# chen-bowen/instacart_next_order_recommendation

Measured on NVIDIA B200. Metric: top-k queries/sec (IR-eval batch: 10,000 queries x 49,688x384 fp32 catalog, top-100), higher is better.
Workload: dtype f32

## Files before the change

### instacart_next_order_recommendation_b200/csrc/gemm_topk.cu

```cuda
#include "select_args.cuh"
#include "select_lean.cuh"
#include "select_finish.cuh"
#include "tc.cuh"

namespace icr {

constexpr int kRingBytes = 192 * 1024;
constexpr int kSegCapMax = 512;
#ifndef ICR_EPI_WARPS_F32
#define ICR_EPI_WARPS_F32 4
#endif
#ifndef ICR_EPI_WARPS_BF16
#define ICR_EPI_WARPS_BF16 8
#endif
__host__ __device__ constexpr int epi_warps(int terms) { return terms == 3 ? ICR_EPI_WARPS_F32 : ICR_EPI_WARPS_BF16; }
constexpr int kEpiWarps = 8;
constexpr int kEpiCols = BN;
constexpr int kGemmThreads = 128 + kEpiWarps * 32;
constexpr int kTmemCols = 512;
constexpr int kMaxStages = 6;
constexpr int kAStatMaxKB = 6;

struct GemmArgs {
  int Q, N;
  int k;
  int kb_per_term;
  int plane_stride;
  int tile_begin, tile_end;
  int chunks;
  int qblocks;
  float acc_scale;
  const float* tau;
  const float* qinv;
// ... 91 lines not shown

template <bool BF16>
__device__ __forceinline__ void filter32(const uint32_t (&r)[32], SegState& s, const float* cinv32, float cmax, float cmin, int rbase,
                                         bool fast, int N, const uint8_t* mask) {
  const float tau_f = unorder_bits(s.tau_ob);
  if (fast) {
    float m[16];
#pragma unroll
    for (int j = 0; j < 16; ++j) m[j] = fmaxf(__uint_as_float(r[2 * j]), __uint_as_float(r[2 * j + 1]));
#pragma unroll
    for (int w = 8; w > 0; w >>= 1)
#pragma unroll
      for (int j = 0; j < w; ++j) m[j] = fmaxf(m[j], m[j + w]);
    const float bound = BF16 ? fmaxf(m[0] * cmax, m[0] * cmin) : m[0];
    if (__any_sync(kFull, bound > tau_f)) {
      float sc[32];
      if (BF16) {
#pragma unroll
        for (int j = 0; j < 32; j += 4) {
          const float4 ci = *reinterpret_cast<const float4*>(cinv32 + j);
          sc[j] = __uint_as_float(r[j]) * ci.x;
          sc[j + 1] = __uint_as_float(r[j + 1]) * ci.y;
          sc[j + 2] = __uint_as_float(r[j + 2]) * ci.z;
          sc[j + 3] = __uint_as_float(r[j + 3]) * ci.w;
        }
      } else {
#pragma unroll
        for (int j = 0; j < 32; ++j) sc[j] = __uint_as_float(r[j]);
      }
      int off[33];
      off[0] = s.cnt;
#pragma unroll
      for (int g = 0; g < 4; ++g) {
        int inc[8];
#pragma unroll
        for (int j = 0; j < 8; ++j) inc[j] = (sc[g * 8 + j] > tau_f) ? 1 : 0;
        const int s01 = inc[0] + inc[1], s23 = inc[2] + inc[3], s45 = inc[4] + inc[5], s67 = inc[6] + inc[7];
        const int b = off[g * 8];
        off[g * 8 + 1] = b + inc[0];
        off[g * 8 + 2] = b + s01;
        off[g * 8 + 3] = b + s01 + inc[2];
        const int b4 = b + s01 + s23;
        off[g * 8 + 4] = b4;
        off[g * 8 + 5] = b4 + inc[4];
        off[g * 8 + 6] = b4 + s45;
        off[g * 8 + 7] = b4 + s45 + inc[6];
        off[g * 8 + 8] = b4 + s45 + s67;
      }
      const uint32_t nrow0 = ~static_cast<uint32_t>(rbase);
#pragma unroll
      for (int j = 0; j < 32; ++j) {
        asm volatile(
            "{\n"
            ".reg .pred p;\n"
            "setp.gt.f32 p, %1, %2;\n"
            "@p st.global.v2.u32 [%0], {%3, %4};\n"
            "}\n" ::"l"(s.seg + off[j]),
            "f"(sc[j]), "f"(tau_f), "r"(nrow0 - j), "r"(__float_as_uint(sc[j]))
            : "memory");
      }
      s.cnt = off[32];
    }
  } else {
#pragma unroll
    for (int j = 0; j < 32; ++j) {
      const int row = rbase + j;
      if (row < N && !(mask && mask[row])) {
        const float sc = BF16 ? __uint_as_float(r[j]) * cinv32[j] : __uint_as_float(r[j]);
        append_if(s, sc, tau_f, ~static_cast<uint32_t>(row));
      }
    }
  }
}

template <bool BF16>
__device__ __forceinline__ void dense_store32(const uint32_t (&r)[32], float* out_row, float qscale, const float* cinv32, int ncols,
// ... 21 lines not shown
    unsigned long long t0, t1;
    asm volatile("mov.u64 %0, %%globaltimer;" : "=l"(t0));
    for (;;) {
      unsigned int v;
      asm volatile("ld.acquire.gpu.global.u32 %0, [%1];" : "=r"(v) : "l"(counter) : "memory");
      if (v >= ctas) break;
      __nanosleep(100);
      asm volatile("mov.u64 %0, %%globaltimer;" : "=l"(t1));
      if (t1 - t0 > 2000000000ull) __trap();
    }
    __threadfence();
  }
  asm volatile("bar.sync 2, %0;" ::"r"(ewarps * 32) : "memory");
}

template <int MODE, bool ASTAT, bool DENSE>
__global__ void __cluster_dims__(2, 1, 1) __launch_bounds__(kGemmThreads, 1)
gemm_topk_kernel(const __grid_constant__ CUtensorMap tma_a, const __grid_constant__ CUtensorMap tma_b, const GemmArgs g) {
  constexpr int TERMS = (MODE == 3) ? 3 : 1;
  static_assert(!ASTAT || TERMS == 1, "A-stationary is a one-term variant");
  constexpr bool BF16 = (MODE == 1);
  constexpr int EW = epi_warps(TERMS), EH = EW / 4, ECOLS = BN / EH;
  constexpr int kStageTiles = ASTAT ? 1 : ((TERMS == 3) ? 4 : 2);
  constexpr int kStageBytes = kStageTiles * kTileBytes;
  constexpr int kAResidentBytes = ASTAT ? kAStatMaxKB * kTileBytes : 0;
  constexpr int kStages = (kRingBytes - kAResidentBytes) / kStageBytes;
  static_assert(kStages <= kMaxStages, "barrier array too small");

  extern __shared__ __align__(1024) unsigned char smem_raw[];
  unsigned char* smem = smem_raw + ((1024u - (smem_u32(smem_raw) & 1023u)) & 1023u);
  unsigned char* a_resident = smem;
  unsigned char* stage_base = smem + kAResidentBytes;
  float* cinv_all = reinterpret_cast<float*>(smem + kRingBytes);
  uint64_t* bars = reinterpret_cast<uint64_t*>(cinv_all + EW * ECOLS);
  uint64_t* full_bar = bars;
  uint64_t* empty_bar = bars + kMaxStages;
  uint64_t* tfull_bar = bars + 2 * kMaxStages;
  uint64_t* tempty_bar = bars + 2 * kMaxStages + 2;
  uint64_t* afull_bar = bars + 2 * kMaxStages + 4;
  uint64_t* aempty_bar = bars + 2 * kMaxStages + 5;
  uint32_t* tmem_ptr = reinterpret_cast<uint32_t*>(bars + 2 * kMaxStages + 6);
  uint32_t* boot_s = reinterpret_cast<uint32_t*>(bars + 2 * kMaxStages + 7);

  const int warp = threadIdx.x >> 5, lane = threadIdx.x & 31;
  const uint32_t rank = cluster_ctarank();
  const int pair = blockIdx.x >> 1, npairs = gridDim.x >> 1;
  const int KB = g.kb_per_term;
  const int items = g.qblocks * g.chunks;

  if (threadIdx.x == 0) {
    for (int s = 0; s < kStages; ++s) {
      mbar_init(smem_u32(&full_bar[s]), 1);
      mbar_init(smem_u32(&empty_bar[s]), 1);
    }
    for (int a = 0; a < 2; ++a) {
      mbar_init(smem_u32(&tfull_bar[a]), 1);
      mbar_init(smem_u32(&tempty_bar[a]), 2 * EW);
    }
    mbar_init(smem_u32(afull_bar), 1);
    mbar_init(smem_u32(aempty_bar), 1);
    asm volatile("fence.mbarrier_init.release.cluster;" ::: "memory");
    asm volatile("prefetch.tensormap [%0];" ::"l"(&tma_a) : "memory");
    asm volatile("prefetch.tensormap [%0];" ::"l"(&tma_b) : "memory");
  }
  if (warp == 2) tmem_alloc_pair(smem_u32(tmem_ptr), kTmemCols);
  tc_fence_before();
  __syncthreads();
  cluster_sync_all();
  tc_fence_after();
  const uint32_t tmem_base = *tmem_ptr;

  if (warp == 0 && lane == 0) {
    int stage = 0;
    uint32_t phase = 0, a_phase = 0;
    for (int pass = g.boot > 0 ? 0 : 1; pass < 2; ++pass)
    for (int w = pair; w < items; w += npairs) {
      const int chunk = w / g.qblocks, qb = w - chunk * g.qblocks;
      const int t0 = chunk_first_tile(g, chunk), t1 = pass == 0 ? t0 + g.boot : chunk_first_tile(g, chunk + 1);
      const int qrow = qb * (2 * BM) + static_cast<int>(rank) * BM;
      if (ASTAT) {
        mbar_wait(smem_u32(aempty_bar), a_phase ^ 1);
        const uint32_t ab = smem_u32(afull_bar);
        if (rank == 0) mbar_expect_tx(ab, 2 * KB * kTileBytes);
        for (int kb = 0; kb < KB; ++kb) tma_load_2d_pair(smem_u32(a_resident + kb * kTileBytes), &tma_a, kb * BK, qrow, ab);
        a_phase ^= 1;
      }
      for (int tile = t0; tile < t1; ++tile) {
        const int crow = tile * BN + static_cast<int>(rank) * BNH;
        for (int kb = 0; kb < KB; ++kb) {
          mbar_wait(smem_u32(&empty_bar[stage]), phase ^ 1);
          const uint32_t fb = smem_u32(&full_bar[stage]);
          if (rank == 0) mbar_expect_tx(fb, 2 * kStageBytes);
          const uint32_t sa = smem_u32(stage_base + stage * kStageBytes);
          if (ASTAT) {
            tma_load_2d_pair(sa, &tma_b, kb * BK, crow, fb);
          } else if (TERMS == 3) {
            tma_load_2d_pair(sa, &tma_a, kb * BK, qrow, fb);
            tma_load_2d_pair(sa + kTileBytes, &tma_a, g.plane_stride + kb * BK, qrow, fb);
            tma_load_2d_pair(sa + 2 * kTileBytes, &tma_b, kb * BK, crow, fb);
            tma_load_2d_pair(sa + 3 * kTileBytes, &tma_b, g.plane_stride + kb * BK, crow, fb);
          } else {
            tma_load_2d_pair(sa, &tma_a, kb * BK, qrow, fb);
            tma_load_2d_pair(sa + kTileBytes, &tma_b, kb * BK, crow, fb);
          }
          if (++stage == kStages) {
            stage = 0;
            phase ^= 1;
          }
        }
      }
    }
  } else if (warp == 1 && rank == 0) {
    const uint32_t fmt = BF16 ? 1u : 0u;
    const uint32_t idesc = (1u << 4) | (fmt << 7) | (fmt << 10) | (static_cast<uint32_t>(BN >> 3) << 17) | (static_cast<uint32_t>((2 * BM) >> 4) << 24);
    const uint64_t a_res0 = smem_desc_sw128(smem_u32(a_resident));
    const uint64_t st0 = smem_desc_sw128(smem_u32(stage_base));
    constexpr uint64_t kTileUnits = kTileBytes >> 4, kStageUnits = kStageBytes >> 4;
    int stage = 0;
    uint32_t phase = 0;
    int acc = 0;
    uint32_t acc_phase = 0, a_phase = 0;
    for (int pass = g.boot > 0 ? 0 : 1; pass < 2; ++pass)
    for (int w = pair; w < items; w += npairs) {
      const int chunk = w / g.qblocks;
      const int t0 = chunk_first_tile(g, chunk), t1 = pass == 0 ? t0 + g.boot : chunk_first_tile(g, chunk + 1);
      if (ASTAT) {
        mbar_wait(smem_u32(afull_bar), a_phase);
        tc_fence_after();
        a_phase ^= 1;
      }
      for (int tile = t0; tile < t1; ++tile) {
        mbar_wait(smem_u32(&tempty_bar[acc]), acc_phase ^ 1);
        tc_fence_after();
        const uint32_t d_tmem = tmem_base + static_cast<uint32_t>(acc * BN);
        for (int kb = 0; kb < KB; ++kb) {
          mbar_wait(smem_u32(&full_bar[stage]), phase);
          tc_fence_after();
          const uint64_t sd = st0 + static_cast<uint64_t>(stage) * kStageUnits;
          if (elect_one()) {
            if (ASTAT) {
              const uint64_t adesc = a_res0 + static_cast<uint64_t>(kb) * kTileUnits, bdesc = sd;
#pragma unroll
              for (int k4 = 0; k4 < BK / 16; ++k4) {
                const uint64_t o = static_cast<uint64_t>(k4 * 2);
                umma_f16_pair(d_tmem, adesc + o, bdesc + o, idesc, (kb | k4) != 0 ? 1u : 0u);
              }
            } else if (TERMS == 3) {
              const uint64_t a_hi = sd, a_lo = sd + kTileUnits, b_hi = sd + 2 * kTileUnits, b_lo = sd + 3 * kTileUnits;
#pragma unroll
              for (int k4 = 0; k4 < BK / 16; ++k4) {
                const uint64_t o = static_cast<uint64_t>(k4 * 2);
                umma_f16_pair(d_tmem, a_hi + o, b_hi + o, idesc, (kb | k4) != 0 ? 1u : 0u);
                umma_f16_pair(d_tmem, a_hi + o, b_lo + o, idesc, 1u);
                umma_f16_pair(d_tmem, a_lo + o, b_hi + o, idesc, 1u);
              }
            } else {
              const uint64_t adesc = sd, bdesc = sd + kTileUnits;
#pragma unroll
              for (int k4 = 0; k4 < BK / 16; ++k4) {
                const uint64_t o = static_cast<uint64_t>(k4 * 2);
                umma_f16_pair(d_tmem, adesc + o, bdesc + o, idesc, (kb | k4) != 0 ? 1u : 0u);
              }
            }
            umma_commit_pair(smem_u32(&empty_bar[stage]));
            if (kb == KB - 1) umma_commit_pair(smem_u32(&tfull_bar[acc]));
          }
          __syncwarp();
          if (++stage == kStages) {
            stage = 0;
            phase ^= 1;
          }
        }
        if (++acc == 2) {
          acc = 0;
          acc_phase ^= 1;
        }
      }
      if (ASTAT) {
        if (elect_one()) umma_commit_pair(smem_u32(aempty_bar));
        __syncwarp();
      }
    }
  } else if (warp >= 4 && warp < 4 + EW) {
    const int ew = (warp - 4) & 3;
    const int half = (warp - 4) >> 2;
    uint64_t* scratch = g.compact_scratch + (static_cast<int64_t>(blockIdx.x) * EW + (warp - 4)) * kSegCapMax;
    float* cinv_s = cinv_all + (warp - 4) * ECOLS;
    const int cap = g.seg_cap;
    int acc = 0;
    uint32_t acc_phase = 0;
    if (!DENSE && g.boot > 0) {
      const int per_tile = g.boot_coarse ? 1 : (ECOLS / 32);
      const int gstride = g.chunks * g.boot * EH * per_tile;
      for (int w = pair; w < items; w += npairs) {
        const int chunk = w / g.qblocks, qb = w - chunk * g.qblocks;
        const int t0 = chunk_first_tile(g, chunk);
        const int q = qb * (2 * BM) + static_cast<int>(rank) * BM + ew * 32 + lane;
        const bool live = q < g.Q;
        float* gq = g.gmax + static_cast<int64_t>(live ? q : 0) * gstride + (chunk * g.boot * EH + half) * per_tile;
        for (int bt = 0; bt < g.boot; ++bt) {
          float m_tile = -INFINITY;
          const int row0 = (t0 + bt) * BN + half * ECOLS;
// ... 28 lines not shown
              }
            }
            m_tile = fmaxf(m_tile, m);
            if (live && !g.boot_coarse) gq[bt * (EH * (ECOLS / 32)) + cb] = m;
          }
          if (live && g.boot_coarse) gq[bt * EH] = m_tile;
          tc_fence_before();
          __syncwarp();
          if (lane == 0) mbar_arrive_cluster(smem_u32(&tempty_bar[acc]), 0);
          if (++acc == 2) {
            acc = 0;
            acc_phase ^= 1;
          }
        }
      }
      k2_grid_barrier(g.gsync, gridDim.x, warp - 4, EW);
      uint32_t* bsc = boot_s + (warp - 4) * (kK2BootCap + kHsBins);
      uint32_t* bhist = bsc + kK2BootCap;
      const int nwarps = static_cast<int>(gridDim.x) * EW;
      for (int j = blockIdx.x * EW + (warp - 4); j < g.Q; j += nwarps) {
        for (int i = lane; i < gstride; i += 32) bsc[i] = order_bits(__ldcg(g.gmax + static_cast<int64_t>(j) * gstride + i));
        __syncwarp();
        uint32_t ks, kr;
        ls_kth(bsc, bsc, gstride, g.k, bhist, lane, ks, kr);
        if (lane == 0) const_cast<float*>(g.tau)[j] = unorder_bits(ks > 1u ? ks - 1u : ks) - g.band;
        __syncwarp();
      }
      k2_grid_barrier(g.gsync + 1, gridDim.x, warp - 4, EW);
    }
    for (int w = pair; w < items; w += npairs) {
      const int chunk = w / g.qblocks, qb = w - chunk * g.qblocks;
      const int t0 = chunk_first_tile(g, chunk), t1 = chunk_first_tile(g, chunk + 1);
      const int q = qb * (2 * BM) + static_cast<int>(rank) * BM + ew * 32 + lane;
      const bool live = q < g.Q;
      const int64_t seg_index = (static_cast<int64_t>(live ? q : 0) * g.chunks + chunk) * EH + half;
      SegState s;
      s.seg = g.cand + seg_index * cap;
      s.cnt = 0;
      constexpr bool dense = DENSE;
      s.tau_ob = (live && !dense) ? order_bits(__ldcg(g.tau + q)) : 0xFFFFFFFFu;
      float* out_q = dense ? g.dense_out + static_cast<int64_t>(live ? q : 0) * g.dense_ld : nullptr;
      const float qscale = dense ? (g.dense_raw ? 1.0f : g.acc_scale * ((BF16 && live) ? g.qinv[q] : 1.0f)) : 0.f;
      const bool vec_ok = dense && (g.dense_ld % 4 == 0) && ((reinterpret_cast<uintptr_t>(g.dense_out) & 15) == 0);
// ... 9 lines not shown
            const float ci = (row0 + i < g.N) ? __ldg(g.cinv + row0 + i) : 0.f;
            cinv_s[i] = ci;
            const float mx = warp_max(ci), mn = -warp_max(-ci);
            if (lane == u) {
              cmax_l = mx;
              cmin_l = mn;
            }
          }
          __syncwarp();
        }
        mbar_wait(smem_u32(&tfull_bar[acc]), acc_phase);
        tc_fence_after();
        const uint32_t taddr = tmem_base + (static_cast<uint32_t>(ew * 32) << 16) + static_cast<uint32_t>(acc * BN + half * ECOLS);
        const bool fast = (row0 + ECOLS <= g.N) && (g.mask == nullptr);
        uint32_t ra[32], rb[32];
        tmem_ld32(taddr, ra);
#pragma unroll 1
        for (int cb = 0; cb < ECOLS / 32; cb += 2) {
          tmem_ld_wait(ra);
          tmem_ld32(taddr + (cb + 1) * 32, rb);
          if (dense) {
            if (live) dense_store32<BF16>(ra, out_q + row0 + cb * 32, qscale, cinv_s + cb * 32, g.N - (row0 + cb * 32), vec_ok);
          } else {
            compact_full_segments(s, scratch, cap, g.k, lane, g.band, g.overflow, q - lane);
            filter32<BF16>(ra, s, cinv_s + cb * 32, __shfl_sync(kFull, cmax_l, cb), __shfl_sync(kFull, cmin_l, cb), row0 + cb * 32, fast,
                           g.N, g.mask);
          }
          tmem_ld_wait(rb);
          if (cb + 2 < ECOLS / 32) tmem_ld32(taddr + (cb + 2) * 32, ra);
          if (dense) {
            if (live) dense_store32<BF16>(rb, out_q + row0 + (cb + 1) * 32, qscale, cinv_s + (cb + 1) * 32, g.N - (row0 + (cb + 1) * 32), vec_ok);
          } else {
            compact_full_segments(s, scratch, cap, g.k, lane, g.band, g.overflow, q - lane);
            filter32<BF16>(rb, s, cinv_s + (cb + 1) * 32, __shfl_sync(kFull, cmax_l, cb + 1), __shfl_sync(kFull, cmin_l, cb + 1),
                           row0 + (cb + 1) * 32, fast, g.N, g.mask);
          }
        }
        tc_fence_before();
        __syncwarp();
        if (lane == 0) mbar_arrive_cluster(smem_u32(&tempty_bar[acc]), 0);
        if (++acc == 2) {
          acc = 0;
          acc_phase ^= 1;
        }
      }
      if (live && !dense) g.cand_cnt[seg_index] = s.cnt;
    }
  }

  tc_fence_before();
  __syncthreads();
// ... 307 lines not shown
          __syncwarp();
          if (++stage == stages) {
            stage = 0;
            phase ^= 1;
          }
        }
        if (++acc == 2) {
          acc = 0;
          acc_phase ^= 1;
        }
      }
    }
  } else if (warp >= 4) {
    const int ew = warp & 3, et = threadIdx.x - 128;
    const int cap = g.seg_cap;
    uint64_t* scratch = g.compact_scratch + (static_cast<int64_t>(blockIdx.x) * kEpiWarps + ew) * kSegCapMax;
    int acc = 0;
    uint32_t acc_phase = 0;
    for (int w = pair; w < items; w += npairs) {
      const int t0 = chunk_first_tile(g, w), t1 = chunk_first_tile(g, w + 1);
      const int64_t seg0 = static_cast<int64_t>(w) * 2 + rank;
      if (g.boot) {
        const int gstride = 4 * static_cast<int>(gridDim.x);
        float best[8];
#pragma unroll
        for (int b = 0; b < 8; ++b) best[b] = -INFINITY;
        for (int bt = 0; bt < g.boot; ++bt) {
          const int row = (t0 + bt) * BN + static_cast<int>(rank) * BNH + ew * 32 + lane;
          const bool valid = row < g.N && !(g.mask && g.mask[row]);
          const float cinv_r = BF16 ? (row < g.N ? __ldg(g.cinv + row) : 0.f) : 1.0f;
          mbar_wait(smem_u32(&tfull_bar[acc]), acc_phase);
// ... 141 lines not shown
  tc_fence_before();
  __syncthreads();
  cluster_sync_all();
  if (warp == 2) {
    tc_fence_after();
    tmem_dealloc_pair(tmem_base, kTmemCols);
  }
}

int launch_row_inv_norms(const void* x, int64_t rows, int64_t dim, int64_t ld, int dtype, float* inv, cudaStream_t st, float* tau_init = nullptr,
                         unsigned int* ovf_init = nullptr);
int launch_split_planes(const float* x, int64_t rows, int64_t dim, int64_t ld, uint16_t* planes, cudaStream_t st);
int launch_screen_plane(const float* x, int64_t rows, int64_t dim, int64_t ld, uint16_t* plane, float* inv, cudaStream_t st, float* tau_init = nullptr,
                        unsigned int* ovf_init = nullptr);

constexpr size_t kGemmSmemBytes = static_cast<size_t>(kRingBytes) + 4 * BN * sizeof(float) +
                                 
                                  (2 * kMaxStages + 6) * sizeof(uint64_t) + 16 + kEpiWarps * (kK2BootCap + kHsBins) * sizeof(uint32_t) + 1024;
static int seg_cap_for(int k) { return k <= 128 ? 288 : kSegCapMax; }
static_assert(kGemmSmemBytes <= 232448, "exceeds the 227 KB of shared memory a CTA may use");
constexpr size_t kSwapSmemBytes = static_cast<size_t>(kRingBytes) + 2 * 256 * 4 + 16 + (2 * kSwapMaxStages + 6) * sizeof(uint64_t) + 16 + kSwapBootBytes + 1024;
static_assert(kSwapSmemBytes <= 232448, "exceeds the 227 KB of shared memory a CTA may use");

static int mode_for(int dtype) { return dtype == ICR_BF16 ? 1 : 2; }
static int carry_cap(int k, int mode) {
  if (mode != 2) return k;
  const int kc = k + (k > 32 ? k : 32);
  return kc < 512 ? kc : 512;
}

static bool swap_applies(int64_t Q, int64_t N, int64_t D) {
  if (Q > 256) return false;
  const int64_t qpad = (Q + 31) / 32 * 32;
  const int64_t kb = (D + BK - 1) / BK;
  const int64_t res = kb * (qpad / 2) * 128;
  const int64_t sweep_bytes = N * ((D + BK - 1) / BK * BK) * 2;
  return res <= (sweep_bytes <= kSmallCatalogBytes ? kSwapResidentMaxSmallCatalog : kSwapResidentMax);
}

// ... 79 lines not shown
    if (e != cudaErrorCooperativeLaunchTooLarge) refused = true;
  }
  kernel<<<grid, threads, smem, st>>>(KArgs(args)...);
}

template <bool DENSE>
static int launch_gemm_variant(int which, int grid, const CUtensorMap& map_a, const CUtensorMap& map_b, const GemmArgs& g, cudaStream_t st) {
  static thread_local SmemAttrCache cache[8];
  int rc = ICR_OK;
#define ICR_SET(ID, K) \
  if (which == ID) rc = ensure_dyn_smem(cache[ID], K, kGemmSmemBytes);
  ICR_GEMM_VARIANTS(ICR_SET, DENSE)
  if constexpr (DENSE) ICR_SET(0, (gemm_topk_kernel<3, false, true>))
#undef ICR_SET
  if (rc) return rc;
  const int terms = which == 0 ? 3 : 1;
  profile_begin(kKernelGemm, terms, st);
  const int threads = 128 + epi_warps(terms) * 32;
#define ICR_RUN(ID, K) \
  if (which == ID) launch_gemm_grid(K, grid, threads, kGemmSmemBytes, st, g.boot > 0, map_a, map_b, g);
  ICR_GEMM_VARIANTS(ICR_RUN, DENSE)
  if constexpr (DENSE) ICR_RUN(0, (gemm_topk_kernel<3, false, true>))
#undef ICR_RUN
  profile_end(st);
  ICR_LAUNCH_CHECK();
  return ICR_OK;
}

static int launch_swap_variant(int which, int grid, const CUtensorMap& map_q, const CUtensorMap& map_c, const GemmArgs& g, cudaStream_t st,
                               const HistSelectArgs& sel = HistSelectArgs{}) {
  static thread_local SmemAttrCache cache[2];
  int rc = ICR_OK;
  if (which == 4) rc = ensure_dyn_smem(cache[0], gemm_swap_kernel<1>, kSwapSmemBytes);
  if (which == 7) rc = ensure_dyn_smem(cache[1], gemm_swap_kernel<2>, kSwapSmemBytes);
  if (rc) return rc;
// ... 28 lines not shown
  int best = c0;
  int64_t best_load = -1;
  for (int c = c0; c <= T && c < c0 + 24; ++c) {
    const int64_t rounds = (static_cast<int64_t>(qblocks) * c + npairs - 1) / npairs;
    const int64_t load = rounds * ((T + c - 1) / c);
    if (best_load < 0 || load < best_load) {
      best_load = load;
      best = c;
    }
  }
  const int64_t want_rows = N * k / kK2BootTarget;
  int tiles = static_cast<int>((want_rows + static_cast<int64_t>(BN) * best - 1) / (static_cast<int64_t>(BN) * best));
  if (tiles < 1) tiles = 1;
  while (best * tiles * (BN / 32) < 2 * k) ++tiles;
  if (best * tiles * (BN / 32) > kK2BootCap) {
    const int eh = epi_warps(1) / 4;
    const int qblocks1 = static_cast<int>((Q + 2 * BM - 1) / (2 * BM));
    int ct = kK2BootCap / (best * eh);
    if (ct > tiles) ct = tiles;
    if (qblocks1 != 1 || T < 2048 || ct < 1 || best * ct * eh < 2 * k) return 0;
    if (static_cast<double>(N) * k / (static_cast<double>(BN) * best * ct) > 2500.0) return 0;
    if (ct * 4 > T / best) return 0;
    if (coarse_out) *coarse_out = 1;
    *chunks_out = best;
    return ct;
  }
  const int64_t dp = (D + 63) / 64 * 64;
  const bool l2_sized = N * dp * 2 <= (96ll << 20);
  if (tiles * (l2_sized ? 2 : 4) > T / best) return 0;
  *chunks_out = best;
  return tiles;
// ... 39 lines not shown
    off += align_up(bytes, 1024);
    return o;
  };
  w.q_planes = take(mode == 2 ? static_cast<size_t>(Q) * dp * 2 : 0);
  w.c_planes = take((mode == 2 && !have_planes) ? static_cast<size_t>(N) * dp * 2 : 0);
  w.qinv = take(static_cast<size_t>(Q) * 4);
  w.cinv = take(!have_cinv ? static_cast<size_t>(N) * 4 : 0);
  w.tau = take(static_cast<size_t>(Q) * 4);
  w.overflow = take(static_cast<size_t>(Q) * 4 + 32);
  w.kc = carry_cap(k, mode);
  for (int i = 0; i < 2; ++i) {
    w.carry[i] = take(static_cast<size_t>(Q) * w.kc * 8);
    w.carry_cnt[i] = take(static_cast<size_t>(Q) * 4);
  }
  w.seg_cap = seg_cap_for(k);
  const int halves = swap ? 2 : epi_warps(1) / 4;
  w.cand = take(static_cast<size_t>(Q) * maxc * halves * w.seg_cap * 8);
  w.cand_cnt = take(static_cast<size_t>(Q) * maxc * halves * 4);
  w.scratch = take(static_cast<size_t>(kNumSMs) * kEpiWarps * kSegCapMax * 8);
  w.dense0 = take(dense0 ? static_cast<size_t>(Q) * dense0_tiles(Q, N) * BN * 4 : 0);
  size_t gmax_bytes = w.boot_pairs ? static_cast<size_t>((Q + 31) / 32 * 32) * 8 * w.boot_pairs * 4 : 0;
  if (w.k2_boot_tiles) gmax_bytes = static_cast<size_t>(Q) * w.k2_boot_chunks * w.k2_boot_tiles * (BN / 32) * 4;
  w.gmax = take(gmax_bytes);
  w.total = off + 1024;
  return w;
}

bool gemm_topk_supported(int64_t Q, int64_t N, int64_t D, int dtype, int k, const uint8_t* mask) {
  (void)mask;
  if (Q < 1 || N < 1 || k > ICR_MAX_K) return false;
  if (dtype == ICR_BF16 && D % 8 != 0) return false;
  if (N > (static_cast<int64_t>(1) << 31) - BN || Q > (static_cast<int64_t>(1) << 30)) return false;
  return true;
}
// ... 125 lines not shown
    return run_select(sp, Q, st);
  }

  if (L.k2_boot_tiles > 0) {
    g.boot = L.k2_boot_tiles;
    g.boot_coarse = L.k2_boot_coarse;
    g.gmax = reinterpret_cast<float*>(base + L.gmax);
    g.gsync = g.overflow + Q;
    g.tile_begin = 0;
    g.tile_end = static_cast<int>((N + BN - 1) / BN);
    g.chunks = L.k2_boot_chunks;
    const int items = qblocks * g.chunks;
    const int pairs = items < kNumSMs / 2 ? items : kNumSMs / 2;
    if ((rc = launch_gemm_variant<false>(which, 2 * pairs, map_a, map_b, g, st))) return rc;
    HistSelectArgs sp = sa;
    sp.nseg = g.chunks * (epi_warps(1) / 4);
    sp.carry_out = mode == 2 ? reinterpret_cast<uint64_t*>(base + L.carry[0]) : nullptr;
    sp.carry_cnt_out = mode == 2 ? reinterpret_cast<int*>(base + L.carry_cnt[0]) : nullptr;
    sp.out_scores = out_scores;
    sp.out_ids = out_ids;
    return run_select(sp, Q, st);
  }

  Phase ph[kMaxPhases];
  const int T = static_cast<int>((N + BN - 1) / BN);
  const bool dense0 = !swap;
  int done_phases = 0;
  if (dense0) {
    const int kDense0Tiles = dense0_tiles(Q, N);
    const int T0 = T < kDense0Tiles ? T : kDense0Tiles;
    float* d0 = reinterpret_cast<float*>(base + L.dense0);
// ... 27 lines not shown
  const int np = plan_phases(N, qblocks, k, ph, kMaxPhases, swap, dense0 ? dense0_tiles(Q, N) : 0);
  for (int pp = 0; pp < np; ++pp) {
    const int p = pp + done_phases;
    g.tile_begin = ph[pp].tile_begin;
    g.tile_end = ph[pp].tile_end;
    g.chunks = ph[pp].chunks;
    const int items = qblocks * g.chunks;
    const int pairs = items < kNumSMs / 2 ? items : kNumSMs / 2;
    const int grid = 2 * pairs;
    if (swap) rc = launch_swap_variant(which, grid, map_a, map_b, g, st);
    else rc = launch_gemm_variant<false>(which, grid, map_a, map_b, g, st);
    if (rc) return rc;
    const bool last = (pp == np - 1);
    const int cur = p & 1, prev = cur ^ 1;
    HistSelectArgs sp = sa;
    sp.nseg = g.chunks * (swap ? 2 : epi_warps(1) / 4);
    sp.carry_in = p > 0 ? reinterpret_cast<uint64_t*>(base + L.carry[prev]) : nullptr;
    sp.carry_cnt_in = p > 0 ? reinterpret_cast<int*>(base + L.carry_cnt[prev]) : nullptr;
    const bool keep = !last || mode == 2;
    sp.carry_out = keep ? reinterpret_cast<uint64_t*>(base + L.carry[cur]) : nullptr;
    sp.carry_cnt_out = keep ? reinterpret_cast<int*>(base + L.carry_cnt[cur]) : nullptr;
    sp.tau_out = last ? nullptr : const_cast<float*>(g.tau);
    sp.out_scores = last ? out_scores : nullptr;
    sp.out_ids = last ? out_ids : nullptr;
    if ((rc = run_select(sp, Q, st))) return rc;
  }
  return ICR_OK;
}

size_t gemm_dense_workspace_bytes(int64_t Qa, int64_t Nb, int64_t D, int dtype) {
  const int64_t dp2 = 2 * ((D + 63) / 64 * 64);
// ... 65 lines not shown
```

Baseline: 15.05 million.

## Use 16 epilogue warps with setmaxnreg split for bf16 top-k path

Makes epilogue warp count a per-variant template: the bf16 top-k path gets 16 filter warps, while control warps shed registers via setmaxnreg and filter warps gain them. The filter loop is split into 16-column halves to cut register pressure, TMEM prefetch is disabled when registers are split, and the boot-stage k-th selection becomes a register-resident radix search instead of a shared-memory histogram. The goal is more epilogue throughput for filtering candidates, at the cost of different segment counts per chunk and serial TMEM loads on that path.

```diff
diff --git a/instacart_next_order_recommendation_b200/csrc/gemm_topk.cu b/instacart_next_order_recommendation_b200/csrc/gemm_topk.cu
--- a/instacart_next_order_recommendation_b200/csrc/gemm_topk.cu
+++ b/instacart_next_order_recommendation_b200/csrc/gemm_topk.cu
@@ -7,16 +7,11 @@
 
 constexpr int kRingBytes = 192 * 1024;
 constexpr int kSegCapMax = 512;
-#ifndef ICR_EPI_WARPS_F32
-#define ICR_EPI_WARPS_F32 4
-#endif
-#ifndef ICR_EPI_WARPS_BF16
-#define ICR_EPI_WARPS_BF16 8
-#endif
-__host__ __device__ constexpr int epi_warps(int terms) { return terms == 3 ? ICR_EPI_WARPS_F32 : ICR_EPI_WARPS_BF16; }
-constexpr int kEpiWarps = 8;
-constexpr int kEpiCols = BN;
-constexpr int kGemmThreads = 128 + kEpiWarps * 32;
+template <int MODE, bool DENSE>
+__host__ __device__ constexpr int epi_warps() { return MODE == 3 ? 4 : ((MODE == 1 && !DENSE) ? 16 : 8); }
+template <int MODE, bool DENSE>
+__host__ __device__ constexpr int gemm_threads() { return 128 + epi_warps<MODE, DENSE>() * 32; }
+constexpr int kEpiWarpsMax = 16;
 constexpr int kTmemCols = 512;
 constexpr int kMaxStages = 6;
 constexpr int kAStatMaxKB = 6;
@@ -138,52 +133,55 @@
       for (int j = 0; j < w; ++j) m[j] = fmaxf(m[j], m[j + w]);
     const float bound = BF16 ? fmaxf(m[0] * cmax, m[0] * cmin) : m[0];
     if (__any_sync(kFull, bound > tau_f)) {
-      float sc[32];
-      if (BF16) {
-#pragma unroll
-        for (int j = 0; j < 32; j += 4) {
-          const float4 ci = *reinterpret_cast<const float4*>(cinv32 + j);
-          sc[j] = __uint_as_float(r[j]) * ci.x;
-          sc[j + 1] = __uint_as_float(r[j + 1]) * ci.y;
-          sc[j + 2] = __uint_as_float(r[j + 2]) * ci.z;
-          sc[j + 3] = __uint_as_float(r[j + 3]) * ci.w;
-        }
-      } else {
-#pragma unroll
-        for (int j = 0; j < 32; ++j) sc[j] = __uint_as_float(r[j]);
-      }
-      int off[33];
-      off[0] = s.cnt;
-#pragma unroll
-      for (int g = 0; g < 4; ++g) {
-        int inc[8];
-#pragma unroll
-        for (int j = 0; j < 8; ++j) inc[j] = (sc[g * 8 + j] > tau_f) ? 1 : 0;
-        const int s01 = inc[0] + inc[1], s23 = inc[2] + inc[3], s45 = inc[4] + inc[5], s67 = inc[6] + inc[7];
-        const int b = off[g * 8];
-        off[g * 8 + 1] = b + inc[0];
-        off[g * 8 + 2] = b + s01;
-        off[g * 8 + 3] = b + s01 + inc[2];
-        const int b4 = b + s01 + s23;
-        off[g * 8 + 4] = b4;
-        off[g * 8 + 5] = b4 + inc[4];
-        off[g * 8 + 6] = b4 + s45;
-        off[g * 8 + 7] = b4 + s45 + inc[6];
-        off[g * 8 + 8] = b4 + s45 + s67;
-      }
       const uint32_t nrow0 = ~static_cast<uint32_t>(rbase);
 #pragma unroll
-      for (int j = 0; j < 32; ++j) {
-        asm volatile(
-            "{\n"
-            ".reg .pred p;\n"
-            "setp.gt.f32 p, %1, %2;\n"
-            "@p st.global.v2.u32 [%0], {%3, %4};\n"
-            "}\n" ::"l"(s.seg + off[j]),
-            "f"(sc[j]), "f"(tau_f), "r"(nrow0 - j), "r"(__float_as_uint(sc[j]))
-            : "memory");
-      }
-      s.cnt = off[32];
+      for (int h = 0; h < 32; h += 16) {
+        float sc[16];
+        if (BF16) {
+#pragma unroll
+          for (int j = 0; j < 16; j += 4) {
+            const float4 ci = *reinterpret_cast<const float4*>(cinv32 + h + j);
+            sc[j] = __uint_as_float(r[h + j]) * ci.x;
+            sc[j + 1] = __uint_as_float(r[h + j + 1]) * ci.y;
+            sc[j + 2] = __uint_as_float(r[h + j + 2]) * ci.z;
+            sc[j + 3] = __uint_as_float(r[h + j + 3]) * ci.w;
+          }
+        } else {
+#pragma unroll
+          for (int j = 0; j < 16; ++j) sc[j] = __uint_as_float(r[h + j]);
+        }
+        int off[17];
+        off[0] = s.cnt;
+#pragma unroll
+        for (int g = 0; g < 2; ++g) {
+          int inc[8];
+#pragma unroll
+          for (int j = 0; j < 8; ++j) inc[j] = (sc[g * 8 + j] > tau_f) ? 1 : 0;
+          const int s01 = inc[0] + inc[1], s23 = inc[2] + inc[3], s45 = inc[4] + inc[5], s67 = inc[6] + inc[7];
+          const int b = off[g * 8];
+          off[g * 8 + 1] = b + inc[0];
+          off[g * 8 + 2] = b + s01;
+          off[g * 8 + 3] = b + s01 + inc[2];
+          const int b4 = b + s01 + s23;
+          off[g * 8 + 4] = b4;
+          off[g * 8 + 5] = b4 + inc[4];
+          off[g * 8 + 6] = b4 + s45;
+          off[g * 8 + 7] = b4 + s45 + inc[6];
+          off[g * 8 + 8] = b4 + s45 + s67;
+        }
+#pragma unroll
+        for (int j = 0; j < 16; ++j) {
+          asm volatile(
+              "{\n"
+              ".reg .pred p;\n"
+              "setp.gt.f32 p, %1, %2;\n"
+              "@p st.global.v2.u32 [%0], {%3, %4};\n"
+              "}\n" ::"l"(s.seg + off[j]),
+              "f"(sc[j]), "f"(tau_f), "r"(nrow0 - (h + j)), "r"(__float_as_uint(sc[j]))
+              : "memory");
+        }
+        s.cnt = off[16];
+      }
     }
   } else {
 #pragma unroll
@@ -235,13 +233,19 @@
   asm volatile("bar.sync 2, %0;" ::"r"(ewarps * 32) : "memory");
 }
 
+constexpr int kCtlRegs = 56, kFilterRegs = 104;
+constexpr size_t kEpiSmemBytes = 4 * BN * sizeof(float);
+
 template <int MODE, bool ASTAT, bool DENSE>
-__global__ void __cluster_dims__(2, 1, 1) __launch_bounds__(kGemmThreads, 1)
+__global__ void __cluster_dims__(2, 1, 1) __launch_bounds__(gemm_threads<MODE, DENSE>(), 1)
 gemm_topk_kernel(const __grid_constant__ CUtensorMap tma_a, const __grid_constant__ CUtensorMap tma_b, const GemmArgs g) {
   constexpr int TERMS = (MODE == 3) ? 3 : 1;
   static_assert(!ASTAT || TERMS == 1, "A-stationary is a one-term variant");
   constexpr bool BF16 = (MODE == 1);
-  constexpr int EW = epi_warps(TERMS), EH = EW / 4, ECOLS = BN / EH;
+  constexpr int EW = epi_warps<MODE, DENSE>(), EH = EW / 4, ECOLS = BN / EH;
+  constexpr bool kRegSplit = EW == 16;
+  constexpr bool kTmemPrefetch = !(BF16 && kRegSplit);
+  static_assert(EW * ECOLS * sizeof(float) <= kEpiSmemBytes && EW <= kEpiWarpsMax, "epilogue buffers");
   constexpr int kStageTiles = ASTAT ? 1 : ((TERMS == 3) ? 4 : 2);
   constexpr int kStageBytes = kStageTiles * kTileBytes;
   constexpr int kAResidentBytes = ASTAT ? kAStatMaxKB * kTileBytes : 0;
@@ -253,7 +257,7 @@
   unsigned char* a_resident = smem;
   unsigned char* stage_base = smem + kAResidentBytes;
   float* cinv_all = reinterpret_cast<float*>(smem + kRingBytes);
-  uint64_t* bars = reinterpret_cast<uint64_t*>(cinv_all + EW * ECOLS);
+  uint64_t* bars = reinterpret_cast<uint64_t*>(smem + kRingBytes + kEpiSmemBytes);
   uint64_t* full_bar = bars;
   uint64_t* empty_bar = bars + kMaxStages;
   uint64_t* tfull_bar = bars + 2 * kMaxStages;
@@ -261,7 +265,6 @@
   uint64_t* afull_bar = bars + 2 * kMaxStages + 4;
   uint64_t* aempty_bar = bars + 2 * kMaxStages + 5;
   uint32_t* tmem_ptr = reinterpret_cast<uint32_t*>(bars + 2 * kMaxStages + 6);
-  uint32_t* boot_s = reinterpret_cast<uint32_t*>(bars + 2 * kMaxStages + 7);
 
   const int warp = threadIdx.x >> 5, lane = threadIdx.x & 31;
   const uint32_t rank = cluster_ctarank();
@@ -290,123 +293,127 @@
   cluster_sync_all();
   tc_fence_after();
   const uint32_t tmem_base = *tmem_ptr;
-
-  if (warp == 0 && lane == 0) {
-    int stage = 0;
-    uint32_t phase = 0, a_phase = 0;
-    for (int pass = g.boot > 0 ? 0 : 1; pass < 2; ++pass)
-    for (int w = pair; w < items; w += npairs) {
-      const int chunk = w / g.qblocks, qb = w - chunk * g.qblocks;
-      const int t0 = chunk_first_tile(g, chunk), t1 = pass == 0 ? t0 + g.boot : chunk_first_tile(g, chunk + 1);
-      const int qrow = qb * (2 * BM) + static_cast<int>(rank) * BM;
-      if (ASTAT) {
-        mbar_wait(smem_u32(aempty_bar), a_phase ^ 1);
-        const uint32_t ab = smem_u32(afull_bar);
-        if (rank == 0) mbar_expect_tx(ab, 2 * KB * kTileBytes);
-        for (int kb = 0; kb < KB; ++kb) tma_load_2d_pair(smem_u32(a_resident + kb * kTileBytes), &tma_a, kb * BK, qrow, ab);
-        a_phase ^= 1;
-      }
-      for (int tile = t0; tile < t1; ++tile) {
-        const int crow = tile * BN + static_cast<int>(rank) * BNH;
-        for (int kb = 0; kb < KB; ++kb) {
-          mbar_wait(smem_u32(&empty_bar[stage]), phase ^ 1);
-          const uint32_t fb = smem_u32(&full_bar[stage]);
-          if (rank == 0) mbar_expect_tx(fb, 2 * kStageBytes);
-          const uint32_t sa = smem_u32(stage_base + stage * kStageBytes);
-          if (ASTAT) {
-            tma_load_2d_pair(sa, &tma_b, kb * BK, crow, fb);
-          } else if (TERMS == 3) {
-            tma_load_2d_pair(sa, &tma_a, kb * BK, qrow, fb);
-            tma_load_2d_pair(sa + kTileBytes, &tma_a, g.plane_stride + kb * BK, qrow, fb);
-            tma_load_2d_pair(sa + 2 * kTileBytes, &tma_b, kb * BK, crow, fb);
-            tma_load_2d_pair(sa + 3 * kTileBytes, &tma_b, g.plane_stride + kb * BK, crow, fb);
-          } else {
-            tma_load_2d_pair(sa, &tma_a, kb * BK, qrow, fb);
-            tma_load_2d_pair(sa + kTileBytes, &tma_b, kb * BK, crow, fb);
-          }
-          if (++stage == kStages) {
-            stage = 0;
-            phase ^= 1;
-          }
-        }
-      }
-    }
-  } else if (warp == 1 && rank == 0) {
-    const uint32_t fmt = BF16 ? 1u : 0u;
-    const uint32_t idesc = (1u << 4) | (fmt << 7) | (fmt << 10) | (static_cast<uint32_t>(BN >> 3) << 17) | (static_cast<uint32_t>((2 * BM) >> 4) << 24);
-    const uint64_t a_res0 = smem_desc_sw128(smem_u32(a_resident));
-    const uint64_t st0 = smem_desc_sw128(smem_u32(stage_base));
-    constexpr uint64_t kTileUnits = kTileBytes >> 4, kStageUnits = kStageBytes >> 4;
-    int stage = 0;
-    uint32_t phase = 0;
-    int acc = 0;
-    uint32_t acc_phase = 0, a_phase = 0;
-    for (int pass = g.boot > 0 ? 0 : 1; pass < 2; ++pass)
-    for (int w = pair; w < items; w += npairs) {
-      const int chunk = w / g.qblocks;
-      const int t0 = chunk_first_tile(g, chunk), t1 = pass == 0 ? t0 + g.boot : chunk_first_tile(g, chunk + 1);
-      if (ASTAT) {
-        mbar_wait(smem_u32(afull_bar), a_phase);
-        tc_fence_after();
-        a_phase ^= 1;
-      }
-      for (int tile = t0; tile < t1; ++tile) {
-        mbar_wait(smem_u32(&tempty_bar[acc]), acc_phase ^ 1);
-        tc_fence_after();
-        const uint32_t d_tmem = tmem_base + static_cast<uint32_t>(acc * BN);
-        for (int kb = 0; kb < KB; ++kb) {
-          mbar_wait(smem_u32(&full_bar[stage]), phase);
+  if (warp < 4) {
+    if (kRegSplit) asm volatile("setmaxnreg.dec.sync.aligned.u32 %0;" ::"n"(kCtlRegs));
+    if (warp == 0 && lane == 0) {
+      int stage = 0;
+      uint32_t phase = 0, a_phase = 0;
+      for (int pass = g.boot > 0 ? 0 : 1; pass < 2; ++pass)
+      for (int w = pair; w < items; w += npairs) {
+        const int chunk = w / g.qblocks, qb = w - chunk * g.qblocks;
+        const int t0 = chunk_first_tile(g, chunk), t1 = pass == 0 ? t0 + g.boot : chunk_first_tile(g, chunk + 1);
+        const int qrow = qb * (2 * BM) + static_cast<int>(rank) * BM;
+        if (ASTAT) {
+          mbar_wait(smem_u32(aempty_bar), a_phase ^ 1);
+          const uint32_t ab = smem_u32(afull_bar);
+          if (rank == 0) mbar_expect_tx(ab, 2 * KB * kTileBytes);
+          for (int kb = 0; kb < KB; ++kb) tma_load_2d_pair(smem_u32(a_resident + kb * kTileBytes), &tma_a, kb * BK, qrow, ab);
+          a_phase ^= 1;
+        }
+        for (int tile = t0; tile < t1; ++tile) {
+          const int crow = tile * BN + static_cast<int>(rank) * BNH;
+          for (int kb = 0; kb < KB; ++kb) {
+            mbar_wait(smem_u32(&empty_bar[stage]), phase ^ 1);
+            const uint32_t fb = smem_u32(&full_bar[stage]);
+            if (rank == 0) mbar_expect_tx(fb, 2 * kStageBytes);
+            const uint32_t sa = smem_u32(stage_base + stage * kStageBytes);
+            if (ASTAT) {
+              tma_load_2d_pair(sa, &tma_b, kb * BK, crow, fb);
+            } else if (TERMS == 3) {
+              tma_load_2d_pair(sa, &tma_a, kb * BK, qrow, fb);
+              tma_load_2d_pair(sa + kTileBytes, &tma_a, g.plane_stride + kb * BK, qrow, fb);
+              tma_load_2d_pair(sa + 2 * kTileBytes, &tma_b, kb * BK, crow, fb);
+              tma_load_2d_pair(sa + 3 * kTileBytes, &tma_b, g.plane_stride + kb * BK, crow, fb);
+            } else {
+              tma_load_2d_pair(sa, &tma_a, kb * BK, qrow, fb);
+              tma_load_2d_pair(sa + kTileBytes, &tma_b, kb * BK, crow, fb);
+            }
+            if (++stage == kStages) {
+              stage = 0;
+              phase ^= 1;
+            }
+          }
+        }
+      }
+    } else if (warp == 1 && rank == 0) {
+      const uint32_t fmt = BF16 ? 1u : 0u;
+      const uint32_t idesc = (1u << 4) | (fmt << 7) | (fmt << 10) | (static_cast<uint32_t>(BN >> 3) << 17) | (static_cast<uint32_t>((2 * BM) >> 4) << 24);
+      const uint64_t a_res0 = smem_desc_sw128(smem_u32(a_resident));
+      const uint64_t st0 = smem_desc_sw128(smem_u32(stage_base));
+      constexpr uint64_t kTileUnits = kTileBytes >> 4, kStageUnits = kStageBytes >> 4;
+      int stage = 0;
+      uint32_t phase = 0;
+      int acc = 0;
+      uint32_t acc_phase = 0, a_phase = 0;
+      for (int pass = g.boot > 0 ? 0 : 1; pass < 2; ++pass)
+      for (int w = pair; w < items; w += npairs) {
+        const int chunk = w / g.qblocks;
+        const int t0 = chunk_first_tile(g, chunk), t1 = pass == 0 ? t0 + g.boot : chunk_first_tile(g, chunk + 1);
+        if (ASTAT) {
+          mbar_wait(smem_u32(afull_bar), a_phase);
           tc_fence_after();
-          const uint64_t sd = st0 + static_cast<uint64_t>(stage) * kStageUnits;
-          if (elect_one()) {
-            if (ASTAT) {
-              const uint64_t adesc = a_res0 + static_cast<uint64_t>(kb) * kTileUnits, bdesc = sd;
-#pragma unroll
-              for (int k4 = 0; k4 < BK / 16; ++k4) {
-                const uint64_t o = static_cast<uint64_t>(k4 * 2);
-                umma_f16_pair(d_tmem, adesc + o, bdesc + o, idesc, (kb | k4) != 0 ? 1u : 0u);
+          a_phase ^= 1;
+        }
+        for (int tile = t0; tile < t1; ++tile) {
+          mbar_wait(smem_u32(&tempty_bar[acc]), acc_phase ^ 1);
+          tc_fence_after();
+          const uint32_t d_tmem = tmem_base + static_cast<uint32_t>(acc * BN);
+          for (int kb = 0; kb < KB; ++kb) {
+            mbar_wait(smem_u32(&full_bar[stage]), phase);
+            tc_fence_after();
+            const uint64_t sd = st0 + static_cast<uint64_t>(stage) * kStageUnits;
+            if (elect_one()) {
+              if (ASTAT) {
+                const uint64_t adesc = a_res0 + static_cast<uint64_t>(kb) * kTileUnits, bdesc = sd;
+  #pragma unroll
+                for (int k4 = 0; k4 < BK / 16; ++k4) {
+                  const uint64_t o = static_cast<uint64_t>(k4 * 2);
+                  umma_f16_pair(d_tmem, adesc + o, bdesc + o, idesc, (kb | k4) != 0 ? 1u : 0u);
+                }
+              } else if (TERMS == 3) {
+                const uint64_t a_hi = sd, a_lo = sd + kTileUnits, b_hi = sd + 2 * kTileUnits, b_lo = sd + 3 * kTileUnits;
+  #pragma unroll
+                for (int k4 = 0; k4 < BK / 16; ++k4) {
+                  const uint64_t o = static_cast<uint64_t>(k4 * 2);
+                  umma_f16_pair(d_tmem, a_hi + o, b_hi + o, idesc, (kb | k4) != 0 ? 1u : 0u);
+                  umma_f16_pair(d_tmem, a_hi + o, b_lo + o, idesc, 1u);
+                  umma_f16_pair(d_tmem, a_lo + o, b_hi + o, idesc, 1u);
+                }
+              } else {
+                const uint64_t adesc = sd, bdesc = sd + kTileUnits;
+  #pragma unroll
+                for (int k4 = 0; k4 < BK / 16; ++k4) {
+                  const uint64_t o = static_cast<uint64_t>(k4 * 2);
+                  umma_f16_pair(d_tmem, adesc + o, bdesc + o, idesc, (kb | k4) != 0 ? 1u : 0u);
+                }
               }
-            } else if (TERMS == 3) {
-              const uint64_t a_hi = sd, a_lo = sd + kTileUnits, b_hi = sd + 2 * kTileUnits, b_lo = sd + 3 * kTileUnits;
-#pragma unroll
-              for (int k4 = 0; k4 < BK / 16; ++k4) {
-                const uint64_t o = static_cast<uint64_t>(k4 * 2);
-                umma_f16_pair(d_tmem, a_hi + o, b_hi + o, idesc, (kb | k4) != 0 ? 1u : 0u);
-                umma_f16_pair(d_tmem, a_hi + o, b_lo + o, idesc, 1u);
-                umma_f16_pair(d_tmem, a_lo + o, b_hi + o, idesc, 1u);
-              }
-            } else {
-              const uint64_t adesc = sd, bdesc = sd + kTileUnits;
-#pragma unroll
-              for (int k4 = 0; k4 < BK / 16; ++k4) {
-                const uint64_t o = static_cast<uint64_t>(k4 * 2);
-                umma_f16_pair(d_tmem, adesc + o, bdesc + o, idesc, (kb | k4) != 0 ? 1u : 0u);
-              }
+              umma_commit_pair(smem_u32(&empty_bar[stage]));
+              if (kb == KB - 1) umma_commit_pair(smem_u32(&tfull_bar[acc]));
             }
-            umma_commit_pair(smem_u32(&empty_bar[stage]));
-            if (kb == KB - 1) umma_commit_pair(smem_u32(&tfull_bar[acc]));
-          }
+            __syncwarp();
+            if (++stage == kStages) {
+              stage = 0;
+              phase ^= 1;
+            }
+          }
+          if (++acc == 2) {
+            acc = 0;
+            acc_phase ^= 1;
+          }
+        }
+        if (ASTAT) {
+          if (elect_one()) umma_commit_pair(smem_u32(aempty_bar));
           __syncwarp();
-          if (++stage == kStages) {
-            stage = 0;
-            phase ^= 1;
-          }
-        }
-        if (++acc == 2) {
-          acc = 0;
-          acc_phase ^= 1;
-        }
-      }
-      if (ASTAT) {
-        if (elect_one()) umma_commit_pair(smem_u32(aempty_bar));
-        __syncwarp();
-      }
-    }
-  } else if (warp >= 4 && warp < 4 + EW) {
-    const int ew = (warp - 4) & 3;
-    const int half = (warp - 4) >> 2;
-    uint64_t* scratch = g.compact_scratch + (static_cast<int64_t>(blockIdx.x) * EW + (warp - 4)) * kSegCapMax;
-    float* cinv_s = cinv_all + (warp - 4) * ECOLS;
+        }
+      }
+    }
+  } else if (warp < 4 + EW) {
+    if (kRegSplit) asm volatile("setmaxnreg.inc.sync.aligned.u32 %0;" ::"n"(kFilterRegs));
+    const int ewi = warp - 4;
+    const int ew = ewi & 3;
+    const int half = ewi >> 2;
+    uint64_t* scratch = g.compact_scratch + (static_cast<int64_t>(blockIdx.x) * kEpiWarpsMax + ewi) * kSegCapMax;
+    float* cinv_s = cinv_all + ewi * ECOLS;
     const int cap = g.seg_cap;
     int acc = 0;
     uint32_t acc_phase = 0;
@@ -465,19 +472,36 @@
           }
         }
       }
-      k2_grid_barrier(g.gsync, gridDim.x, warp - 4, EW);
-      uint32_t* bsc = boot_s + (warp - 4) * (kK2BootCap + kHsBins);
-      uint32_t* bhist = bsc + kK2BootCap;
+      k2_grid_barrier(g.gsync, gridDim.x, ewi, EW);
       const int nwarps = static_cast<int>(gridDim.x) * EW;
-      for (int j = blockIdx.x * EW + (warp - 4); j < g.Q; j += nwarps) {
-        for (int i = lane; i < gstride; i += 32) bsc[i] = order_bits(__ldcg(g.gmax + static_cast<int64_t>(j) * gstride + i));
-        __syncwarp();
-        uint32_t ks, kr;
-        ls_kth(bsc, bsc, gstride, g.k, bhist, lane, ks, kr);
+      const int fold = (g.boot_coarse && EH > 2) ? EH / 2 : 1, nrank = gstride / fold;
+      for (int j = blockIdx.x * EW + ewi; j < g.Q; j += nwarps) {
+        uint32_t v[kK2BootCap / 32];
+#pragma unroll
+        for (int u = 0; u < kK2BootCap / 32; ++u) {
+          const int i = u * 32 + lane;
+          v[u] = 0u;
+          if (i < nrank) {
+            const float* src = g.gmax + static_cast<int64_t>(j) * gstride + i * fold;
+            float m = __ldcg(src);
+            for (int f = 1; f < fold; ++f) m = fmaxf(m, __ldcg(src + f));
+            v[u] = order_bits(m);
+          }
+        }
+        uint32_t ks = 0u;
+        int need = g.k;
+        for (int b = 31; b >= 0; --b) {
+          const uint32_t hi = (ks >> b) | 1u;
+          int c = 0;
+#pragma unroll
+          for (int u = 0; u < kK2BootCap / 32; ++u) c += (v[u] >> b) == hi ? 1 : 0;
+          c = __reduce_add_sync(kFull, c);
+          if (c >= need) ks |= 1u << b;
+          else need -= c;
+        }
         if (lane == 0) const_cast<float*>(g.tau)[j] = unorder_bits(ks > 1u ? ks - 1u : ks) - g.band;
-        __syncwarp();
-      }
-      k2_grid_barrier(g.gsync + 1, gridDim.x, warp - 4, EW);
+      }
+      k2_grid_barrier(g.gsync + 1, gridDim.x, ewi, EW);
     }
     for (int w = pair; w < items; w += npairs) {
       const int chunk = w / g.qblocks, qb = w - chunk * g.qblocks;
@@ -517,6 +541,16 @@
         const uint32_t taddr = tmem_base + (static_cast<uint32_t>(ew * 32) << 16) + static_cast<uint32_t>(acc * BN + half * ECOLS);
         const bool fast = (row0 + ECOLS <= g.N) && (g.mask == nullptr);
         uint32_t ra[32], rb[32];
+        if (!kTmemPrefetch) {
+#pragma unroll 1
+          for (int cb = 0; cb < ECOLS / 32; ++cb) {
+            tmem_ld32(taddr + cb * 32, ra);
+            tmem_ld_wait(ra);
+            compact_full_segments(s, scratch, cap, g.k, lane, g.band, g.overflow, q - lane);
+            filter32<BF16>(ra, s, cinv_s + cb * 32, __shfl_sync(kFull, cmax_l, cb), __shfl_sync(kFull, cmin_l, cb), row0 + cb * 32, fast,
+                           g.N, g.mask);
+          }
+        } else {
         tmem_ld32(taddr, ra);
 #pragma unroll 1
         for (int cb = 0; cb < ECOLS / 32; cb += 2) {
@@ -538,6 +572,7 @@
             filter32<BF16>(rb, s, cinv_s + (cb + 1) * 32, __shfl_sync(kFull, cmax_l, cb + 1), __shfl_sync(kFull, cmin_l, cb + 1),
                            row0 + (cb + 1) * 32, fast, g.N, g.mask);
           }
+        }
         }
         tc_fence_before();
         __syncwarp();
@@ -875,7 +910,7 @@
   } else if (warp >= 4) {
     const int ew = warp & 3, et = threadIdx.x - 128;
     const int cap = g.seg_cap;
-    uint64_t* scratch = g.compact_scratch + (static_cast<int64_t>(blockIdx.x) * kEpiWarps + ew) * kSegCapMax;
+    uint64_t* scratch = g.compact_scratch + (static_cast<int64_t>(blockIdx.x) * kEpiWarpsMax + ew) * kSegCapMax;
     int acc = 0;
     uint32_t acc_phase = 0;
     for (int w = pair; w < items; w += npairs) {
@@ -1047,15 +1082,14 @@
 int launch_screen_plane(const float* x, int64_t rows, int64_t dim, int64_t ld, uint16_t* plane, float* inv, cudaStream_t st, float* tau_init = nullptr,
                         unsigned int* ovf_init = nullptr);
 
-constexpr size_t kGemmSmemBytes = static_cast<size_t>(kRingBytes) + 4 * BN * sizeof(float) +
-                                 
-                                  (2 * kMaxStages + 6) * sizeof(uint64_t) + 16 + kEpiWarps * (kK2BootCap + kHsBins) * sizeof(uint32_t) + 1024;
+constexpr size_t kGemmSmemBytes = static_cast<size_t>(kRingBytes) + kEpiSmemBytes + (2 * kMaxStages + 6) * sizeof(uint64_t) + 16 + 1024;
 static int seg_cap_for(int k) { return k <= 128 ? 288 : kSegCapMax; }
 static_assert(kGemmSmemBytes <= 232448, "exceeds the 227 KB of shared memory a CTA may use");
 constexpr size_t kSwapSmemBytes = static_cast<size_t>(kRingBytes) + 2 * 256 * 4 + 16 + (2 * kSwapMaxStages + 6) * sizeof(uint64_t) + 16 + kSwapBootBytes + 1024;
 static_assert(kSwapSmemBytes <= 232448, "exceeds the 227 KB of shared memory a CTA may use");
 
 static int mode_for(int dtype) { return dtype == ICR_BF16 ? 1 : 2; }
+static int topk_segs_per_chunk(int mode) { return (mode == 1 ? epi_warps<1, false>() : epi_warps<2, false>()) / 4; }
 static int carry_cap(int k, int mode) {
   if (mode != 2) return k;
   const int kc = k + (k > 32 ? k : 32);
@@ -1165,11 +1199,10 @@
   if constexpr (DENSE) ICR_SET(0, (gemm_topk_kernel<3, false, true>))
 #undef ICR_SET
   if (rc) return rc;
-  const int terms = which == 0 ? 3 : 1;
-  profile_begin(kKernelGemm, terms, st);
-  const int threads = 128 + epi_warps(terms) * 32;
+  profile_begin(kKernelGemm, which == 0 ? 3 : 1, st);
+  auto kernel_threads = [](int id) { return id == 0 ? gemm_threads<3, true>() : id <= 2 ? gemm_threads<1, DENSE>() : gemm_threads<2, DENSE>(); };
 #define ICR_RUN(ID, K) \
-  if (which == ID) launch_gemm_grid(K, grid, threads, kGemmSmemBytes, st, g.boot > 0, map_a, map_b, g);
+  if (which == ID) launch_gemm_grid(K, grid, kernel_threads(ID), kGemmSmemBytes, st, g.boot > 0, map_a, map_b, g);
   ICR_GEMM_VARIANTS(ICR_RUN, DENSE)
   if constexpr (DENSE) ICR_RUN(0, (gemm_topk_kernel<3, false, true>))
 #undef ICR_RUN
@@ -1228,7 +1261,7 @@
   if (tiles < 1) tiles = 1;
   while (best * tiles * (BN / 32) < 2 * k) ++tiles;
   if (best * tiles * (BN / 32) > kK2BootCap) {
-    const int eh = epi_warps(1) / 4;
+    const int eh = 2;
     const int qblocks1 = static_cast<int>((Q + 2 * BM - 1) / (2 * BM));
     int ct = kK2BootCap / (best * eh);
     if (ct > tiles) ct = tiles;
@@ -1298,10 +1331,10 @@
     w.carry_cnt[i] = take(static_cast<size_t>(Q) * 4);
   }
   w.seg_cap = seg_cap_for(k);
-  const int halves = swap ? 2 : epi_warps(1) / 4;
-  w.cand = take(static_cast<size_t>(Q) * maxc * halves * w.seg_cap * 8);
-  w.cand_cnt = take(static_cast<size_t>(Q) * maxc * halves * 4);
-  w.scratch = take(static_cast<size_t>(kNumSMs) * kEpiWarps * kSegCapMax * 8);
+  const int segs = swap ? 2 : topk_segs_per_chunk(mode);
+  w.cand = take(static_cast<size_t>(Q) * maxc * segs * w.seg_cap * 8);
+  w.cand_cnt = take(static_cast<size_t>(Q) * maxc * segs * 4);
+  w.scratch = take(static_cast<size_t>(kNumSMs) * kEpiWarpsMax * kSegCapMax * 8);
   w.dense0 = take(dense0 ? static_cast<size_t>(Q) * dense0_tiles(Q, N) * BN * 4 : 0);
   size_t gmax_bytes = w.boot_pairs ? static_cast<size_t>((Q + 31) / 32 * 32) * 8 * w.boot_pairs * 4 : 0;
   if (w.k2_boot_tiles) gmax_bytes = static_cast<size_t>(Q) * w.k2_boot_chunks * w.k2_boot_tiles * (BN / 32) * 4;
@@ -1457,7 +1490,7 @@
     const int pairs = items < kNumSMs / 2 ? items : kNumSMs / 2;
     if ((rc = launch_gemm_variant<false>(which, 2 * pairs, map_a, map_b, g, st))) return rc;
     HistSelectArgs sp = sa;
-    sp.nseg = g.chunks * (epi_warps(1) / 4);
+    sp.nseg = g.chunks * topk_segs_per_chunk(mode);
     sp.carry_out = mode == 2 ? reinterpret_cast<uint64_t*>(base + L.carry[0]) : nullptr;
     sp.carry_cnt_out = mode == 2 ? reinterpret_cast<int*>(base + L.carry_cnt[0]) : nullptr;
     sp.out_scores = out_scores;
@@ -1515,7 +1548,7 @@
     const bool last = (pp == np - 1);
     const int cur = p & 1, prev = cur ^ 1;
     HistSelectArgs sp = sa;
-    sp.nseg = g.chunks * (swap ? 2 : epi_warps(1) / 4);
+    sp.nseg = g.chunks * (swap ? 2 : topk_segs_per_chunk(mode));
     sp.carry_in = p > 0 ? reinterpret_cast<uint64_t*>(base + L.carry[prev]) : nullptr;
     sp.carry_cnt_in = p > 0 ? reinterpret_cast<int*>(base + L.carry_cnt[prev]) : nullptr;
     const bool keep = !last || mode == 2;
```

Result: slower. 14.11 million, median of 6 (-6.2%).
